# dronefreak/CABiNet

Measured on AMD Instinct MI355X. Metric: 1024x1024 images/sec fwd+bwd (CABiNet-MobileNetV3-Large), higher is better.
Workload: dtype f32; 1 GPU; BASELINE configs[2]: CABiNet-MobileNetV3-Large, 8x3x1024x1024 synthetic 8-class per GPU, fwd + 2x OhemCE + bwd + grad all-reduce + SGD step, HIP CAB/FFM kernels, fp32, random-init (model seed 0, gamma=0.5); per_gpu_batch=8, global_batch=8, n_classes=8, parallelism=dp1, miopen_find_mode=FAST

## Files before the change

cabinet_amd/_lib.py:

```python

from __future__ import annotations

import ctypes
import os
import threading

_PKG_DIR = os.path.dirname(os.path.abspath(__file__))
LIB_PATH = os.path.join(_PKG_DIR, "libcabinet_hip.so")
ABI_VERSION = 8

_c_float_p = ctypes.c_void_p
_INT, _FLT, _SZ, _PTR = ctypes.c_int, ctypes.c_float, ctypes.c_size_t, ctypes.c_void_p

SIGNATURES = {
    "cabinet_abi_version": (_INT, []),
    "cabinet_last_error": (ctypes.c_char_p, []),
    "cabinet_cab_attn_supported": (_INT, [_INT] * 2),
    "cabinet_cab_attn_precision_supported": (_INT, [_INT] * 3),
    "cabinet_cab_attn_fwd_workspace_bytes": (_SZ, [_INT] * 5),
    "cabinet_cab_attn_fwd": (_INT, [_PTR, _PTR, _PTR, _FLT, _INT, _INT, _INT, _INT, _INT, _PTR, _PTR, _PTR, _SZ, _PTR]),
    "cabinet_cab_attn_proj_supported": (_INT, [_INT] * 5),
    "cabinet_cab_attn_proj_fwd": (_INT, [_PTR] * 4 + [_FLT] + [_INT] * 5 + [_PTR] * 3 + [_PTR]),
    "cabinet_cab_attn_bwd_workspace_bytes": (_SZ, [_INT] * 4),
    "cabinet_cab_attn_bwd": (_INT, [_PTR] * 6 + [_FLT] + [_INT] * 4 + [_PTR] * 3 + [_PTR, _SZ, _PTR]),
# ... 20 lines not shown
                            + [_PTR, _SZ, _PTR]),
    "cabinet_cab_qkv_bwd_workspace_bytes": (_SZ, [_INT] * 7 + [_PTR]),
    "cabinet_cab_qkv_bwd": (_INT, [_PTR] * 20 + [_INT] * 7 + [_PTR] + [_INT] + [_PTR] * 9 + [_PTR, _SZ, _PTR]),
    "cabinet_conv1x1_fwd_workspace_bytes": (_SZ, [_INT] * 2),
    "cabinet_conv1x1_fwd": (_INT, [_PTR] * 2 + [_INT] * 4 + [_PTR] + [_PTR, _SZ, _PTR]),
    "cabinet_conv1x1_bias_supported": (_INT, [_INT] * 4),
    "cabinet_conv1x1_bias_fwd": (_INT, [_PTR] * 3 + [_INT] * 4 + [_PTR] + [_PTR, _SZ, _PTR]),
    "cabinet_channel_sum": (_INT, [_PTR] + [_INT] * 3 + [_PTR] + [_PTR]),
    "cabinet_conv1x1_bwd_workspace_bytes": (_SZ, [_INT] * 4),
    "cabinet_conv1x1_bwd": (_INT, [_PTR] * 3 + [_INT] * 4 + [_PTR] * 2 + [_PTR, _SZ, _PTR]),
    "cabinet_bn_act_workspace_bytes": (_SZ, [_INT] * 3),
    "cabinet_bn_act_fwd": (_INT, [_PTR] * 6 + [_INT] * 5 + [_FLT, _FLT] + [_PTR] * 3 + [_PTR, _SZ, _PTR]),
    "cabinet_bn_act_bwd": (_INT, [_PTR] * 6 + [_INT] * 5 + [_PTR] * 3 + [_PTR, _SZ, _PTR]),
    "cabinet_bn_cls_supported": (_INT, [_INT] * 3),
    "cabinet_bn_cls_table_floats": (_INT, [_INT] * 2),
    "cabinet_bn_cls_fwd_workspace_bytes": (_SZ, [_INT] * 3),
    "cabinet_bn_cls_fwd": (_INT, [_PTR] * 8 + [_INT] * 6 + [_FLT, _FLT] + [_PTR] * 2 + [_PTR, _SZ, _PTR]),
    "cabinet_bn_cls_bwd_workspace_bytes": (_SZ, [_INT] * 4),
    "cabinet_bn_cls_bwd": (_INT, [_PTR] * 3 + [_INT] * 6 + [_PTR] * 5 + [_PTR, _SZ, _PTR]),
    "cabinet_gate_act_fwd": (_INT, [_PTR] * 2 + [_INT] * 4 + [_PTR] + [_PTR]),
    "cabinet_gate_act_bwd_workspace_bytes": (_SZ, [_INT] * 3),
    "cabinet_gate_act_bwd": (_INT, [_PTR] * 3 + [_INT] * 4 + [_PTR] * 2 + [_PTR, _SZ, _PTR]),
    "cabinet_bn_dwconv_fwd_workspace_bytes": (_SZ, [_INT] * 4),
    "cabinet_bn_dwconv_fwd": (_INT, [_PTR] * 6 + [_INT] * 8 + [_FLT, _FLT] + [_PTR] * 3 + [_PTR, _SZ, _PTR]),
    "cabinet_bn_dwconv_bwd_workspace_bytes": (_SZ, [_INT] * 6),
    "cabinet_bn_dwconv_bwd": (_INT, [_PTR] * 7 + [_INT] * 8 + [_PTR] * 4 + [_PTR, _SZ, _PTR]),
    "cabinet_stem_conv_fwd": (_INT, [_PTR] * 2 + [_INT] * 3 + [_PTR] + [_PTR]),
    "cabinet_stem_conv_wrw_workspace_bytes": (_SZ, [_INT] * 3),
    "cabinet_stem_conv_wrw": (_INT, [_PTR] * 2 + [_INT] * 3 + [_PTR] + [_PTR, _SZ, _PTR]),
    "cabinet_pwconv_supported": (_INT, [_INT] * 3),
    "cabinet_pwconv_fwd": (_INT, [_PTR] * 2 + [_INT] * 4 + [_PTR] + [_PTR]),
    "cabinet_pwconv_bwd_workspace_bytes": (_SZ, [_INT] * 4),
    "cabinet_pwconv_bwd": (_INT, [_PTR] * 3 + [_INT] * 4 + [_PTR] * 2 + [_PTR, _SZ, _PTR]),
    "cabinet_bn_act_fwd_part": (_INT, [_PTR] * 7 + [_INT] * 6 + [_FLT, _FLT] + [_PTR] * 3 + [_PTR]),
    "cabinet_conv3x3_supported": (_INT, [_INT] * 3),
    "cabinet_conv3x3_tile_blocks": (_INT, [_INT] * 3),
    "cabinet_conv3x3_fwd_workspace_bytes": (_SZ, [_INT] * 6),
    "cabinet_conv3x3_fwd": (_INT, [_PTR] * 3 + [_INT] * 6 + [_PTR] * 2 + [_PTR, _SZ, _PTR]),
    "cabinet_conv3x3_bwd_workspace_bytes": (_SZ, [_INT] * 6),
    "cabinet_conv3x3_bwd": (_INT, [_PTR] * 4 + [_INT] * 6 + [_PTR] * 3 + [_PTR, _SZ, _PTR]),
    "cabinet_dwconv_supported": (_INT, [_INT] * 2),
    "cabinet_dwconv_fwd": (_INT, [_PTR] * 2 + [_INT] * 6 + [_PTR] + [_PTR]),
    "cabinet_dwconv_bwd_workspace_bytes": (_SZ, [_INT] * 6),
    "cabinet_dwconv_bwd": (_INT, [_PTR] * 3 + [_INT] * 6 + [_PTR] * 2 + [_PTR, _SZ, _PTR]),
    "cabinet_cab_local_supported": (_INT, [_INT] * 4),
    "cabinet_cab_local_fwd_workspace_bytes": (_SZ, [_INT] * 4),
    "cabinet_cab_local_bwd_workspace_bytes": (_SZ, [_INT] * 4),
    "cabinet_cab_local_fwd": (_INT, [_PTR] * 3 + [_PTR] * 5 + [_INT] * 5 + [_FLT, _FLT] + [_PTR] * 3 + [_PTR, _SZ, _PTR]),
    "cabinet_cab_local_bwd": (_INT, [_PTR] * 4 + [_PTR] * 3 + [_PTR] * 2 + [_INT] * 5 + [_PTR] * 3 + [_PTR] * 3 + [_PTR, _SZ, _PTR]),
    "cabinet_eval_chip_accum_supported": (_INT, [_INT] * 6),
    "cabinet_eval_chip_accum": (_INT, [_PTR] * 2 + [_INT] * 6 + [_PTR] + [_INT] * 4 + [_PTR] * 2 + [_PTR]),
    "cabinet_eval_scale_merge": (_INT, [_PTR] + [_INT] * 8 + [_PTR] + [_INT] * 2 + [_PTR]),
    "cabinet_eval_argmax_hist": (_INT, [_PTR] * 2 + [_INT] * 5 + [_PTR] * 2 + [_PTR]),
    "cabinet_se_act_bwd_workspace_bytes": (_SZ, [_INT] * 3),
    "cabinet_se_act_bwd_reduce": (_INT, [_PTR] * 8 + [_INT] * 4 + [_PTR] * 2 + [_PTR, _SZ, _PTR]),
    "cabinet_se_act_bwd_coef": (_INT, [_PTR] * 3 + [_INT] * 4 + [_PTR] * 4 + [_PTR]),
    "cabinet_se_act_bwd_dx": (_INT, [_PTR] * 9 + [_INT] * 4 + [_PTR] + [_PTR]),
}

_lock = threading.Lock()
_lib = None


def _preload_hip_runtime():
    import sys

# ... 48 lines not shown
```

cabinet_amd/build.py:

```python

from __future__ import annotations

import argparse
import hashlib
import os
import shutil
import subprocess
import sys
from concurrent.futures import ThreadPoolExecutor

PKG_DIR = os.path.dirname(os.path.abspath(__file__))
CSRC = os.path.join(PKG_DIR, "csrc")
OBJ_DIR = os.path.join(PKG_DIR, "csrc", "build")
LIB_PATH = os.path.join(PKG_DIR, "libcabinet_hip.so")
ARCH = "gfx950"

SOURCES = ["capi.hip", "cab_attn_fwd.hip", "cab_attn_bf16.hip", "cab_attn_bwd.hip", "ffm.hip", "ffm_bwd_fused.hip", "ffm_bwd_adj.hip", "ffm_fwd_fused.hip", "gemm_bf16.hip", "ohem.hip", "cab_local.hip", "cab_local_tiled.hip", "cab_qkv.hip", "cab_qkv_fused.hip", "bn_act.hip", "dwconv.hip", "stem_conv.hip", "pwconv.hip", "small_gemm.hip", "conv3x3_wino.hip", "bn_cls.hip", "eval_tail.hip"]
HEADERS = ["common.hpp", "cab_local.hpp", "cab_qkv.hpp", "blocks.hpp", "act.hpp", "bn_finalize.hpp", os.path.join("..", "..", "include", "cabinet_hip.h")]


def _hipcc():
    for cand in (os.environ.get("HIPCC"), shutil.which("hipcc"), "/opt/rocm/bin/hipcc"):
        if cand and os.path.exists(cand):
            return cand
    raise RuntimeError("hipcc not found: cannot build libcabinet_hip.so")


def _digest(paths):
    h = hashlib.sha256()
    for p in paths:
        with open(p, "rb") as f:
            h.update(f.read())
    return h.hexdigest()


def source_digest():
    paths = [os.path.join(CSRC, s) for s in SOURCES] + [os.path.normpath(os.path.join(CSRC, h)) for h in HEADERS]
    return _digest(paths)


def is_fresh():
    stamp = LIB_PATH + ".stamp"
    if not (os.path.exists(LIB_PATH) and os.path.exists(stamp)):
        return False
    with open(stamp) as f:
        return f.read().strip() == _stamp()


def _stamp():
    return (source_digest() + " " + os.environ.get("CABINET_EXTRA_HIPCC_FLAGS", "").strip()).strip()
# ... 46 lines not shown
```

cabinet_amd/csrc/capi.hip:

```cpp
#include "../../include/cabinet_hip.h"

#include <stdarg.h>
#include <stdint.h>
#include <stdio.h>

#include "blocks.hpp"
#include "cab_local.hpp"
#include "cab_qkv.hpp"
#include "common.hpp"

namespace cabinet {
int attn_fwd_kvsplit(int B, int n);
bool attn_shape_supported(int Kc, int Vc);
hipError_t attn_fwd_dispatch(const float* q, const float* k, const float* v, float scale, int B, int Kc,
                             int Vc, int n, float* ctx, float* lse, float* part_ctx, float* part_lse,
                             int kvsplit, hipStream_t stream);
bool attn_fwd_proj_supported(int B, int Kc, int Vc, int Co, int n);
hipError_t attn_fwd_proj_dispatch(const float* q, const float* k, const float* v, const float* w_out, float scale, int B, int Kc,
                                  int Vc, int Co, int n, float* ctx, float* glob, float* lse, hipStream_t stream);
bool attn_bf16_supported(int Kc, int Vc);
size_t attn_bf16_pack_bytes(int B, int Kc, int Vc, int n, int precision);
hipError_t attn_fwd_bf16_dispatch(const float* q, const float* k, const float* v, float scale, int B, int Kc, int Vc, int n,
                                  float* ctx, float* lse, float* part_ctx, float* part_lse, int kvsplit, void* pack, int precision,
                                  hipStream_t stream);
// ... 53 lines not shown
size_t gate_act_workspace(int rows, int P);
hipError_t gate_act_fwd_run(const float* x, const float* gate, int rows, int P, int act, float* y, hipStream_t stream);
hipError_t gate_act_bwd_run(const float* dy, const float* x, const float* gate, int rows, int P, int act, float* dx,
                            float* dgate, void* ws, hipStream_t stream);
bool bn_cls_supported(int C, int K, int P);
int bn_cls_table_floats(int C, int K);
size_t bn_cls_fwd_workspace(int B, int C, int P);
size_t bn_cls_bwd_workspace(int B, int C, int K, int P);
hipError_t bn_cls_fwd_run(const float* z, const float* conv_part, const float* bn_w, const float* bn_b, float* run_mean, float* run_var,
                          const float* w_cls, const float* bias, int B, int C, int K, int H, int W, int training, float momentum,
                          float eps, float* y, float* tab, void* ws, hipStream_t stream);
hipError_t bn_cls_bwd_run(const float* dy, const float* z, const float* tab, int B, int C, int K, int H, int W, int training, float* dz,
                          float* dbn_w, float* dbn_b, float* dw_cls, float* dbias, void* ws, hipStream_t stream);
bool dwconv_supported(int K, int S);
size_t dwconv_bwd_workspace(int B, int C, int H, int W, int K);
hipError_t dwconv_fwd_run(const float* x, const float* w, int B, int C, int H, int W, int K, int S, float* y,
                          hipStream_t stream);
hipError_t dwconv_bwd_run(const float* dy, const float* x, const float* w, int B, int C, int H, int W, int K, int S,
                          float* dx, float* dw, void* ws, hipStream_t stream);
size_t bn_dwconv_fwd_workspace(int B, int C, int H, int W);
size_t bn_dwconv_bwd_workspace(int B, int C, int H, int W, int K);
hipError_t bn_dwconv_fwd_run(const float* z, const float* bn_w, const float* bn_b, float* run_mean, float* run_var,
                             const float* w, int B, int C, int H, int W, int K, int S, int act, int training,
                             float momentum, float eps, float* y, float* save_mean, float* save_invstd, void* ws,
                             hipStream_t stream);
hipError_t bn_dwconv_bwd_run(const float* dy, const float* z, const float* bn_w, const float* bn_b,
                             const float* save_mean, const float* save_invstd, const float* w, int B, int C, int H,
                             int W, int K, int S, int act, int training, float* dz, float* dbn_w, float* dbn_b,
                             float* dw, void* ws, hipStream_t stream);
size_t stem_conv_wrw_workspace(int B, int H, int W);
hipError_t stem_conv_fwd_run(const float* x, const float* w, int B, int H, int W, float* y, hipStream_t stream);
hipError_t stem_conv_wrw_run(const float* dy, const float* x, int B, int H, int W, float* dw, void* ws,
                             hipStream_t stream);
bool pwconv_supported(int Ci, int Co, int P);
size_t pwconv_bwd_workspace(int B, int Ci, int Co, int P);
hipError_t pwconv_fwd_run(const float* x, const float* w, int B, int Ci, int Co, int P, float* y, hipStream_t stream);
hipError_t pwconv_bwd_run(const float* dy, const float* x, const float* w, int B, int Ci, int Co, int P, float* dx,
                          float* dw, void* ws, hipStream_t stream);
int ohem_blocks(int B, int H, int W);
hipError_t ohem_up_fwd_run(int nh, const float* const* low, const long long* labels, int B, int C, int Hl, int Wl, int H, int W,
                           float thresh, int ignore_lb, float* const* loss_px, float* const* blk_sum, int* const* blk_cnt,
                           hipStream_t stream);
hipError_t ohem_stats_run(const float* blk_sum, const int* blk_cnt, int nheads, int nblk, double* stats, hipStream_t stream);
size_t ohem_up_bwd_workspace(int B, int C, int H, int Wl);
bool ohem_up_supported(int C, int Wl, int W);
hipError_t ohem_up_bwd_run(int nh, const float* const* low, const long long* labels, const float* const* loss_px, int B, int C,
                           int Hl, int Wl, int H, int W, float thresh, int ignore_lb, float coef, float* dlow, void* ws,
                           hipStream_t stream);
struct WinoShape {
    int B, C0, C1, K, H, W;
};
bool conv3x3_supported(int C0, int C1, int K);
bool conv3x3_shape_ok(const WinoShape& s);
int conv3x3_tile_blocks(int B, int H, int W);
size_t conv3x3_fwd_workspace(const WinoShape& s);
size_t conv3x3_bwd_workspace(const WinoShape& s);
hipError_t conv3x3_fwd_run(const WinoShape& s, const float* x0, const float* x1, const float* w, float* y, float* stat_part, void* ws,
                           hipStream_t stream);
hipError_t conv3x3_bwd_run(const WinoShape& s, const float* dy, const float* x0, const float* x1, const float* w, float* dx0,
                           float* dx1, float* dw, void* ws, hipStream_t stream);
int eval_chip_threads(int C, int wl, int cw, int nsrc);
hipError_t eval_chip_accum_run(const float* a, const float* b, int N, int C, int hl, int wl, int ch, int cw, float* dst, int FH,
                               int FW, int y0, int x0, const float* rcp_y, const float* rcp_x, hipStream_t stream);
hipError_t eval_scale_merge_run(const float* prob, int N, int C, int FH, int FW, int hst, int hed, int wst, int wed, float* total,
                                int H, int W, hipStream_t stream);
hipError_t eval_argmax_hist_run(const float* total, const long long* labels, int N, int C, int H, int W, int ignore_lb, long long* hist,
// ... 865 lines not shown
    if (B <= 0 || Ci <= 0 || Co <= 0 || P <= 0) return fail(CABINET_ERR_INVALID_ARG, "%s: non-positive dimension", who);
    if (!cabinet::pwconv_supported(Ci, Co, P))
        return fail(CABINET_ERR_UNSUPPORTED, "%s: Ci=%d, Co=%d (multiples of 8, <= 120, block product <= 8)", who, Ci, Co);
    return CABINET_OK;
}

int cabinet_pwconv_supported(int Ci, int Co, int P) {
    return Ci > 0 && Co > 0 && P > 0 && cabinet::pwconv_supported(Ci, Co, P) ? 1 : 0;
}

int cabinet_pwconv_fwd(const float* x, const float* w, int B, int Ci, int Co, int P, float* y, cabinet_stream_t stream) {
    if (int rc = check_pwconv(B, Ci, Co, P, "pwconv_fwd")) return rc;
    if (!x || !w || !y) return fail(CABINET_ERR_INVALID_ARG, "pwconv_fwd: null tensor pointer");
    return hip_status(cabinet::pwconv_fwd_run(x, w, B, Ci, Co, P, y, static_cast<hipStream_t>(stream)),
                      "pwconv_fwd launch");
}

size_t cabinet_pwconv_bwd_workspace_bytes(int B, int Ci, int Co, int P) {
    if (B <= 0 || Ci <= 0 || Co <= 0 || P <= 0 || !cabinet::pwconv_supported(Ci, Co, P)) return 0;
    return cabinet::pwconv_bwd_workspace(B, Ci, Co, P);
}

int cabinet_pwconv_bwd(const float* dy, const float* x, const float* w, int B, int Ci, int Co, int P, float* dx,
                       float* dw, void* workspace, size_t workspace_bytes, cabinet_stream_t stream) {
    if (int rc = check_pwconv(B, Ci, Co, P, "pwconv_bwd")) return rc;
    if (!dy || !x || !w) return fail(CABINET_ERR_INVALID_ARG, "pwconv_bwd: null tensor pointer");
    const size_t need = cabinet::pwconv_bwd_workspace(B, Ci, Co, P);
    if (dw && (!workspace || workspace_bytes < need))
        return fail(CABINET_ERR_WORKSPACE, "pwconv_bwd: workspace %zu < %zu bytes", workspace_bytes, need);
    return hip_status(cabinet::pwconv_bwd_run(dy, x, w, B, Ci, Co, P, dx, dw, workspace, static_cast<hipStream_t>(stream)),
                      "pwconv_bwd launch");
}

static int check_conv3x3(const cabinet::WinoShape& s, const char* who) {
    if (s.B <= 0 || s.C0 <= 0 || s.C1 < 0 || s.K <= 0 || s.H <= 0 || s.W <= 0)
        return fail(CABINET_ERR_INVALID_ARG, "%s: non-positive dimension", who);
    if (!cabinet::conv3x3_shape_ok(s))
        return fail(CABINET_ERR_UNSUPPORTED,
                    "%s: C0=%d C1=%d Co=%d H=%d W=%d (C0, C1 multiples of 16; Co, C0+C1 multiples of 64; C0 %% 64 == 0 when C1 > 0; "
                    "one image's tensors < 1 GiB)", who, s.C0, s.C1, s.K, s.H, s.W);
    return CABINET_OK;
}

int cabinet_conv3x3_supported(int C0, int C1, int Co) { return cabinet::conv3x3_supported(C0, C1, Co) ? 1 : 0; }

int cabinet_conv3x3_tile_blocks(int B, int H, int W) {
    return B > 0 && H > 0 && W > 0 ? cabinet::conv3x3_tile_blocks(B, H, W) : 0;
}

size_t cabinet_conv3x3_fwd_workspace_bytes(int B, int C0, int C1, int Co, int H, int W) {
    const cabinet::WinoShape s{B, C0, C1, Co, H, W};
    return B > 0 && H > 0 && W > 0 && cabinet::conv3x3_shape_ok(s) ? cabinet::conv3x3_fwd_workspace(s) : 0;
}

int cabinet_conv3x3_fwd(const float* x0, const float* x1, const float* w, int B, int C0, int C1, int Co, int H, int W, float* y,
                        float* bn_part, void* workspace, size_t workspace_bytes, cabinet_stream_t stream) {
    const cabinet::WinoShape s{B, C0, C1, Co, H, W};
    if (int rc = check_conv3x3(s, "conv3x3_fwd")) return rc;
    if (!x0 || !w || !y || (C1 > 0 && !x1)) return fail(CABINET_ERR_INVALID_ARG, "conv3x3_fwd: null tensor pointer");
    CABINET_REQUIRE_ALIGNED("conv3x3_fwd", x0, x1, w, y, bn_part);
    const size_t need = cabinet::conv3x3_fwd_workspace(s);
    if (!workspace || workspace_bytes < need)
        return fail(CABINET_ERR_WORKSPACE, "conv3x3_fwd: workspace %zu < %zu bytes", workspace_bytes, need);
    return hip_status(cabinet::conv3x3_fwd_run(s, x0, C1 > 0 ? x1 : nullptr, w, y, bn_part, workspace, static_cast<hipStream_t>(stream)),
                      "conv3x3_fwd launch");
}
// ... 68 lines not shown
```

cabinet_amd/functional.py:

```python

from __future__ import annotations

import ctypes as _ct

import torch
import torch.nn.functional as F

from . import _lib


def _ptr(t):
    return t.data_ptr() if t is not None else None


def _stream_handle(device):
    return torch.cuda.current_stream(device).cuda_stream


def _workspace(nbytes, device):
    if nbytes == 0:
        return None, 0
    ws = torch.empty(nbytes, dtype=torch.uint8, device=device)
    return ws, nbytes

# ... 1283 lines not shown
        with torch.cuda.device(x.device):
            rc = lib.cabinet_pwconv_fwd(_ptr(x), _ptr(w2), B, Ci, Co, P, _ptr(y), _stream_handle(x.device))
        _lib.check(rc, "cabinet_pwconv_fwd")
        fn_ctx.save_for_backward(x, w2)
        fn_ctx.w_shape = weight.shape
        return y

    @staticmethod
    @torch.amp.custom_bwd(device_type="cuda")
    def backward(fn_ctx, g):
        lib = _lib.load()
        x, w2 = fn_ctx.saved_tensors
        g = _f32c(g)
        Co, Ci = w2.shape
        B, P = x.shape[0], x.shape[2] * x.shape[3]
        dx = torch.empty_like(x) if fn_ctx.needs_input_grad[0] else None
        dw = torch.empty_like(w2) if fn_ctx.needs_input_grad[1] else None
        ws, nbytes = _workspace(lib.cabinet_pwconv_bwd_workspace_bytes(B, Ci, Co, P), x.device)
        with torch.cuda.device(x.device):
            rc = lib.cabinet_pwconv_bwd(_ptr(g), _ptr(x), _ptr(w2), B, Ci, Co, P, _ptr(dx), _ptr(dw), _ptr(ws), nbytes,
                                        _stream_handle(x.device))
        _lib.check(rc, "cabinet_pwconv_bwd")
        return dx, (dw.view(fn_ctx.w_shape) if dw is not None else None)


def pwconv(x, conv):
    if not x.is_cuda:
        raise RuntimeError("pwconv: device tensors only")
    return _PwConv.apply(x, conv.weight)




def eval_chip_accum_supported(logits, chip_size, flip=False):
    if not (logits.is_cuda and logits.dim() == 4 and _lib.available()):
        return False
    _, C, hl, wl = logits.shape
    return bool(_lib.load().cabinet_eval_chip_accum_supported(C, hl, wl, int(chip_size[0]), int(chip_size[1]), int(bool(flip))))


def eval_chip_accum(dst, logits, logits_flipped, chip_size, origin, rcp_y=None, rcp_x=None):
    lib = _lib.load()
    if not (dst.is_cuda and dst.dtype == torch.float32 and dst.is_contiguous()):
        raise RuntimeError("eval_chip_accum: dst must be a dense fp32 device tensor")
    a = _f32c(logits)
    b = _f32c(logits_flipped) if logits_flipped is not None else None
    if b is not None and b.shape != a.shape:
        raise RuntimeError("eval_chip_accum: the flipped chip's logits must have the shape of the chip's")
    N, C, hl, wl = a.shape
    if dst.shape[:2] != (N, C):
        raise RuntimeError(f"eval_chip_accum: dst {tuple(dst.shape)} does not match logits {tuple(a.shape)}")
    FH, FW = dst.shape[2:]
    ry = _f32c(rcp_y) if rcp_y is not None else None
    rx = _f32c(rcp_x) if rcp_x is not None else None
    if (ry is not None and ry.numel() != FH) or (rx is not None and rx.numel() != FW):
        raise RuntimeError("eval_chip_accum: rcp_y / rcp_x must have one entry per row / column of dst")
    dev = dst.device
    with torch.cuda.device(dev):
        rc = lib.cabinet_eval_chip_accum(_ptr(a), _ptr(b), N, C, hl, wl, int(chip_size[0]), int(chip_size[1]), _ptr(dst), FH, FW,
                                         int(origin[0]), int(origin[1]), _ptr(ry), _ptr(rx), _stream_handle(dev))
    _lib.check(rc, "cabinet_eval_chip_accum")
    return dst


def eval_scale_merge_supported(total):
    return bool(total.is_cuda and total.dim() == 4 and _lib.available() and total.shape[0] * total.shape[1] <= 65535
# ... 43 lines not shown
```

cabinet_amd/models/cabinet.py:

```python

from __future__ import annotations

import logging
from pathlib import Path
from typing import Optional, Tuple

import torch
import torch.nn as nn
import torch.nn.functional as F

from .. import functional as _functional
from ..functional import (batched_bn_counters, bn_act, bn_relu_cls, conv1x1, conv1x1_bias_supported, conv3x3, conv3x3_bn_part,
                          conv3x3_supported, ffm_fused, ffm_fused_upsampled, stem_conv, stem_conv_supported)
from .cab import ContextAggregationBlock
from .constants import MODEL_CONFIG, MOBILENETV3_CFGS
from .mobilenetv3 import MobileNetV3

logger = logging.getLogger(__name__)


def _resize(x, size):
    return F.interpolate(x, size=size, mode="bilinear", align_corners=False)


def _is_plain_3x3(conv: nn.Conv2d) -> bool:
    return (conv.kernel_size == (3, 3) and conv.stride == (1, 1) and conv.padding == (1, 1) and conv.dilation == (1, 1) and
            conv.groups == 1 and conv.bias is None and conv.padding_mode == "zeros")


def _conv3x3_bn_relu(conv: nn.Conv2d, bn: nn.BatchNorm2d, x: torch.Tensor, x1: Optional[torch.Tensor] = None) -> torch.Tensor:
    c1 = 0 if x1 is None else x1.shape[1]
    if _functional.CONV3X3_ENABLED and _is_plain_3x3(conv) and conv3x3_supported(x.shape[1], c1, conv.out_channels, x.shape[2], x.shape[3]):
        part = conv3x3_bn_part(x, conv.out_channels) if bn.training else None
        return bn_act(conv3x3(x, conv.weight, x1, part), bn, "relu", conv_part=part)
    return bn_act(conv(x if x1 is None else torch.cat([x, x1], dim=1)), bn, "relu")


def _conv3x3_bn_relu_cls(conv: nn.Conv2d, bn: nn.BatchNorm2d, cls: nn.Conv2d, x: torch.Tensor,
                         x1: Optional[torch.Tensor] = None) -> torch.Tensor:
    c1 = 0 if x1 is None else x1.shape[1]
    if _functional.CONV3X3_ENABLED and _is_plain_3x3(conv) and conv3x3_supported(x.shape[1], c1, conv.out_channels, x.shape[2], x.shape[3]):
        part = conv3x3_bn_part(x, conv.out_channels) if bn.training else None
        return bn_relu_cls(conv3x3(x, conv.weight, x1, part), bn, cls, conv_part=part)
    return bn_relu_cls(conv(x if x1 is None else torch.cat([x, x1], dim=1)), bn, cls)


class ConvBNReLU(nn.Module):

    def __init__(self, in_chan: int, out_chan: int, kernel_size: int = 3, stride: int = 1, padding: int = 1,
                 dilation: int = 1):
        super().__init__()
        self.conv = nn.Conv2d(in_chan, out_chan, kernel_size, stride, padding, dilation=dilation, bias=False)
        self.bn = nn.BatchNorm2d(out_chan)
        self.relu = nn.ReLU(inplace=True)
        self.init_weight()

    def forward(self, x: torch.Tensor) -> torch.Tensor:
        if not x.is_cuda:
            return self.relu(self.bn(self.conv(x)))
        if x.shape[1] == 3 and stem_conv_supported(self.conv):
            return bn_act(stem_conv(x, self.conv), self.bn, "relu")
        return _conv3x3_bn_relu(self.conv, self.bn, x)

    def init_weight(self) -> None:
        nn.init.kaiming_normal_(self.conv.weight, a=1)
        if self.conv.bias is not None:
            nn.init.constant_(self.conv.bias, 0)

# ... 146 lines not shown
```

cabinet_amd/models/mobilenetv3.py:

```python

from __future__ import annotations

import math
from pathlib import Path

import torch
import torch.nn as nn

__all__ = ["MobileNetV3", "InvertedResidual", "SELayer", "HardSwish", "HardSigmoid",
           "mobilenetv3_large", "mobilenetv3_small"]


def _make_divisible(v, divisor, min_value=None):
    floor = divisor if min_value is None else min_value
    rounded = max(floor, int(v + divisor / 2) // divisor * divisor)
    return rounded + divisor if rounded < 0.9 * v else rounded


class HardSigmoid(nn.Module):

    def __init__(self, inplace: bool = True) -> None:
        super().__init__()
        self.relu = nn.ReLU6(inplace=inplace)

# ... 10 lines not shown
    def forward(self, x):
        return x * self.sigmoid(x)


class SELayer(nn.Module):

    def __init__(self, channel, reduction=4):
        super().__init__()
        squeezed = _make_divisible(channel // reduction, 8)
        self.avg_pool = nn.AdaptiveAvgPool2d(1)
        self.fc = nn.Sequential(nn.Linear(channel, squeezed), nn.ReLU(inplace=True),
                                nn.Linear(squeezed, channel), HardSigmoid())

    def gate(self, x):
        n, c = x.shape[:2]
        return self.fc(self.avg_pool(x).view(n, c))

    def forward(self, x):
        n, c = x.shape[:2]
        return x * self.gate(x).view(n, c, 1, 1)


def _act(use_hs):
    return HardSwish() if use_hs else nn.ReLU(inplace=True)


class _FusedSequential(nn.Sequential):

    def forward(self, x, residual=None):
        if not x.is_cuda:
            y = super().forward(x)
            return y if residual is None else residual + y
        from ..functional import (bn_act, bn_act_dwconv, dwconv, dwconv_supported, gate_act, pwconv,
                                  pwconv_supported, se_tail)

        layers = [m for m in self if not isinstance(m, nn.Identity)]

        def act_of(m):
            return "relu" if isinstance(m, nn.ReLU) else "hardswish" if isinstance(m, HardSwish) else None

        i = 0
        while i < len(layers):
            m = layers[i]
            nxt = layers[i + 1] if i + 1 < len(layers) else None
            if isinstance(m, nn.BatchNorm2d) and isinstance(nxt, SELayer):
                act = act_of(layers[i + 2]) if i + 2 < len(layers) else None
                x, i = se_tail(x, m, nxt, act), i + (3 if act else 2)
            elif isinstance(m, nn.BatchNorm2d):
                act = act_of(nxt)
                nxt2 = layers[i + 2] if act and i + 2 < len(layers) else None
                if isinstance(nxt2, nn.Conv2d) and nxt2.groups > 1 and dwconv_supported(nxt2):
                    x, i = bn_act_dwconv(x, m, act, nxt2), i + 3
                else:
                    last = i + (2 if act else 1) >= len(layers)
                    x, i = bn_act(x, m, act, residual if last else None), i + (2 if act else 1)
                    if last:
                        residual = None
            elif isinstance(m, SELayer):
                act = act_of(nxt)
                x, i = gate_act(x, m.gate(x), act), i + (2 if act else 1)
            elif isinstance(m, nn.Conv2d) and m.groups == 1 and pwconv_supported(m, x):
                x, i = pwconv(x, m), i + 1
            elif isinstance(m, nn.Conv2d) and m.groups > 1 and dwconv_supported(m):
                x, i = dwconv(x, m), i + 1
            else:
                x, i = m(x), i + 1
        return x if residual is None else residual + x


def conv_3x3_bn(inp, oup, stride):
    return _FusedSequential(nn.Conv2d(inp, oup, 3, stride, 1, bias=False), nn.BatchNorm2d(oup), HardSwish())


def conv_1x1_bn(inp, oup):
    return _FusedSequential(nn.Conv2d(inp, oup, 1, 1, 0, bias=False), nn.BatchNorm2d(oup), HardSwish())


class InvertedResidual(nn.Module):

    def __init__(self, inp, hidden_dim, oup, kernel_size, stride, use_se, use_hs):
        super().__init__()
        if stride not in (1, 2):
            raise ValueError(f"stride must be 1 or 2, got {stride}")
        self.identity = stride == 1 and inp == oup
        pad = (kernel_size - 1) // 2

        def depthwise():
            return nn.Conv2d(hidden_dim, hidden_dim, kernel_size, stride, pad, groups=hidden_dim, bias=False)

        layers = []
        if inp == hidden_dim:
            layers += [depthwise(), nn.BatchNorm2d(hidden_dim), _act(use_hs)]
            layers += [SELayer(hidden_dim) if use_se else nn.Identity()]
        else:
            layers += [nn.Conv2d(inp, hidden_dim, 1, 1, 0, bias=False), nn.BatchNorm2d(hidden_dim), _act(use_hs)]
            layers += [depthwise(), nn.BatchNorm2d(hidden_dim)]
            layers += [SELayer(hidden_dim) if use_se else nn.Identity(), _act(use_hs)]
# ... 75 lines not shown
```

include/cabinet_hip.h:

```cpp
#ifndef CABINET_HIP_H_
#define CABINET_HIP_H_

#include <stddef.h>

#ifdef __cplusplus
extern "C" {
#endif

#define CABINET_ABI_VERSION 8

#define CABINET_OK 0
#define CABINET_ERR_INVALID_ARG (-1)
#define CABINET_ERR_UNSUPPORTED (-2)
#define CABINET_ERR_WORKSPACE (-3)
#define CABINET_ERR_HIP (-4)

typedef void* cabinet_stream_t;

int cabinet_abi_version(void);
const char* cabinet_last_error(void);

#define CABINET_PREC_FP32 0
#define CABINET_PREC_BF16X3 1
#define CABINET_PREC_BF16X6 2
// ... 181 lines not shown
int cabinet_se_act_bwd_reduce(const float* dy, const float* z, const float* mean, const float* invstd, const float* bn_weight,
                              const float* bn_bias, const float* gate, const float* a2, int B, int C, int P, int act,
                              float* sums, float* da2, void* workspace, size_t workspace_bytes, cabinet_stream_t stream);
int cabinet_se_act_bwd_coef(const float* sums, const float* gate, const float* ds, int B, int C, int P, int training,
                            float* dbn_weight, float* dbn_bias, float* coef, float* ds_over_p, cabinet_stream_t stream);
int cabinet_se_act_bwd_dx(const float* dy, const float* z, const float* mean, const float* invstd, const float* bn_weight,
                          const float* bn_bias, const float* gate, const float* ds_over_p, const float* coef,
                          int B, int C, int P, int act, float* dz, cabinet_stream_t stream);

size_t cabinet_bn_dwconv_fwd_workspace_bytes(int B, int C, int H, int W);
int cabinet_bn_dwconv_fwd(const float* z, const float* bn_weight, const float* bn_bias,
                          float* running_mean, float* running_var, const float* conv_weight,
                          int B, int C, int H, int W, int K, int stride, int act, int training,
                          float momentum, float eps, float* y, float* save_mean, float* save_invstd,
                          void* workspace, size_t workspace_bytes, cabinet_stream_t stream);
size_t cabinet_bn_dwconv_bwd_workspace_bytes(int B, int C, int H, int W, int K, int stride);
int cabinet_bn_dwconv_bwd(const float* dy, const float* z, const float* bn_weight, const float* bn_bias,
                          const float* save_mean, const float* save_invstd, const float* conv_weight,
                          int B, int C, int H, int W, int K, int stride, int act, int training,
                          float* dz, float* dbn_weight, float* dbn_bias, float* dconv_weight,
                          void* workspace, size_t workspace_bytes, cabinet_stream_t stream);

int cabinet_stem_conv_fwd(const float* x, const float* weight, int B, int H, int W, float* y, cabinet_stream_t stream);
size_t cabinet_stem_conv_wrw_workspace_bytes(int B, int H, int W);
int cabinet_stem_conv_wrw(const float* dy, const float* x, int B, int H, int W, float* dw,
                          void* workspace, size_t workspace_bytes, cabinet_stream_t stream);

int cabinet_pwconv_supported(int Ci, int Co, int P);
int cabinet_pwconv_fwd(const float* x, const float* w, int B, int Ci, int Co, int P, float* y, cabinet_stream_t stream);
size_t cabinet_pwconv_bwd_workspace_bytes(int B, int Ci, int Co, int P);
int cabinet_pwconv_bwd(const float* dy, const float* x, const float* w, int B, int Ci, int Co, int P,
                       float* dx, float* dw, void* workspace, size_t workspace_bytes, cabinet_stream_t stream);

int cabinet_conv3x3_supported(int C0, int C1, int Co);
int cabinet_conv3x3_tile_blocks(int B, int H, int W);
size_t cabinet_conv3x3_fwd_workspace_bytes(int B, int C0, int C1, int Co, int H, int W);
int cabinet_conv3x3_fwd(const float* x0, const float* x1, const float* w, int B, int C0, int C1, int Co, int H, int W,
                        float* y, float* bn_part, void* workspace, size_t workspace_bytes, cabinet_stream_t stream);
size_t cabinet_conv3x3_bwd_workspace_bytes(int B, int C0, int C1, int Co, int H, int W);
int cabinet_conv3x3_bwd(const float* dy, const float* x0, const float* x1, const float* w, int B, int C0, int C1, int Co,
                        int H, int W, float* dx0, float* dx1, float* dw,
                        void* workspace, size_t workspace_bytes, cabinet_stream_t stream);

int cabinet_eval_chip_accum_supported(int C, int hl, int wl, int ch, int cw, int flip);
int cabinet_eval_chip_accum(const float* a, const float* b, int N, int C, int hl, int wl, int ch, int cw, float* dst, int FH, int FW,
                            int y0, int x0, const float* rcp_y, const float* rcp_x, cabinet_stream_t stream);
int cabinet_eval_scale_merge(const float* prob, int N, int C, int FH, int FW, int hst, int hed, int wst, int wed, float* total, int H,
                             int W, cabinet_stream_t stream);
int cabinet_eval_argmax_hist(const float* total, const long long* labels, int N, int C, int H, int W, int ignore_lb, long long* hist,
                             unsigned char* pred, cabinet_stream_t stream);

#ifdef __cplusplus
}
#endif
#endif
```

Before: 340.3 images/s.

## Add split-K MFMA weight-gradient kernel for wide pointwise convolutions

Adds a custom HIP kernel for the weight gradient of 1x1 convolutions that pwconv does not cover. It splits the pixel dimension across many workgroups, each accumulating an fp32 MFMA tile into a per-split slab, and a second kernel sums the slabs. Forward and input-gradient still go through MIOpen; only dW replaces MIOpen's wrw path, which is likely slow for tall-skinny reductions at 1024x1024. This adds a workspace of nsplit*Co*Ci floats and an extra reduction launch.

After: 351.2 images/s, median of 6. 3.2% higher.

```diff
diff --git a/cabinet_amd/_lib.py b/cabinet_amd/_lib.py
--- a/cabinet_amd/_lib.py
+++ b/cabinet_amd/_lib.py
@@ -76,6 +76,9 @@
     "cabinet_pwconv_fwd": (_INT, [_PTR] * 2 + [_INT] * 4 + [_PTR] + [_PTR]),
     "cabinet_pwconv_bwd_workspace_bytes": (_SZ, [_INT] * 4),
     "cabinet_pwconv_bwd": (_INT, [_PTR] * 3 + [_INT] * 4 + [_PTR] * 2 + [_PTR, _SZ, _PTR]),
+    "cabinet_pwconv_wide_supported": (_INT, [_INT] * 3),
+    "cabinet_pwconv_wide_wgrad_workspace_bytes": (_SZ, [_INT] * 4),
+    "cabinet_pwconv_wide_wgrad": (_INT, [_PTR] * 2 + [_INT] * 4 + [_PTR] + [_PTR, _SZ, _PTR]),
     "cabinet_bn_act_fwd_part": (_INT, [_PTR] * 7 + [_INT] * 6 + [_FLT, _FLT] + [_PTR] * 3 + [_PTR]),
     "cabinet_conv3x3_supported": (_INT, [_INT] * 3),
     "cabinet_conv3x3_tile_blocks": (_INT, [_INT] * 3),
diff --git a/cabinet_amd/build.py b/cabinet_amd/build.py
--- a/cabinet_amd/build.py
+++ b/cabinet_amd/build.py
@@ -15,7 +15,7 @@
 LIB_PATH = os.path.join(PKG_DIR, "libcabinet_hip.so")
 ARCH = "gfx950"
 
-SOURCES = ["capi.hip", "cab_attn_fwd.hip", "cab_attn_bf16.hip", "cab_attn_bwd.hip", "ffm.hip", "ffm_bwd_fused.hip", "ffm_bwd_adj.hip", "ffm_fwd_fused.hip", "gemm_bf16.hip", "ohem.hip", "cab_local.hip", "cab_local_tiled.hip", "cab_qkv.hip", "cab_qkv_fused.hip", "bn_act.hip", "dwconv.hip", "stem_conv.hip", "pwconv.hip", "small_gemm.hip", "conv3x3_wino.hip", "bn_cls.hip", "eval_tail.hip"]
+SOURCES = ["capi.hip", "cab_attn_fwd.hip", "cab_attn_bf16.hip", "cab_attn_bwd.hip", "ffm.hip", "ffm_bwd_fused.hip", "ffm_bwd_adj.hip", "ffm_fwd_fused.hip", "gemm_bf16.hip", "ohem.hip", "cab_local.hip", "cab_local_tiled.hip", "cab_qkv.hip", "cab_qkv_fused.hip", "bn_act.hip", "dwconv.hip", "stem_conv.hip", "pwconv.hip", "pwconv_wide.hip", "small_gemm.hip", "conv3x3_wino.hip", "bn_cls.hip", "eval_tail.hip"]
 HEADERS = ["common.hpp", "cab_local.hpp", "cab_qkv.hpp", "blocks.hpp", "act.hpp", "bn_finalize.hpp", os.path.join("..", "..", "include", "cabinet_hip.h")]
 
 
diff --git a/cabinet_amd/csrc/capi.hip b/cabinet_amd/csrc/capi.hip
--- a/cabinet_amd/csrc/capi.hip
+++ b/cabinet_amd/csrc/capi.hip
@@ -109,6 +109,10 @@
 hipError_t stem_conv_fwd_run(const float* x, const float* w, int B, int H, int W, float* y, hipStream_t stream);
 hipError_t stem_conv_wrw_run(const float* dy, const float* x, int B, int H, int W, float* dw, void* ws,
                              hipStream_t stream);
+bool pwconv_wide_supported(int Ci, int Co, int P);
+size_t pwconv_wide_wgrad_workspace(int B, int Ci, int Co, int P);
+hipError_t pwconv_wide_wgrad_run(const float* dy, const float* x, int B, int Ci, int Co, int P, float* dw, void* ws,
+                                 hipStream_t stream);
 bool pwconv_supported(int Ci, int Co, int P);
 size_t pwconv_bwd_workspace(int B, int Ci, int Co, int P);
 hipError_t pwconv_fwd_run(const float* x, const float* w, int B, int Ci, int Co, int P, float* y, hipStream_t stream);
@@ -1040,6 +1044,33 @@
                       "pwconv_bwd launch");
 }
 
+int cabinet_pwconv_wide_supported(int Ci, int Co, int P) {
+    return Ci > 0 && Co > 0 && P > 0 && cabinet::pwconv_wide_supported(Ci, Co, P) ? 1 : 0;
+}
+
+size_t cabinet_pwconv_wide_wgrad_workspace_bytes(int B, int Ci, int Co, int P) {
+    if (B <= 0 || Ci <= 0 || Co <= 0 || P <= 0 || !cabinet::pwconv_wide_supported(Ci, Co, P)) return 0;
+    if ((long long)B * ((P + 63) / 64) > (1ll << 30)) return 0;
+    return cabinet::pwconv_wide_wgrad_workspace(B, Ci, Co, P);
+}
+
+int cabinet_pwconv_wide_wgrad(const float* dy, const float* x, int B, int Ci, int Co, int P, float* dw, void* workspace,
+                              size_t workspace_bytes, cabinet_stream_t stream) {
+    if (B <= 0 || Ci <= 0 || Co <= 0 || P <= 0)
+        return fail(CABINET_ERR_INVALID_ARG, "pwconv_wide_wgrad: non-positive dimension");
+    if ((long long)B * ((P + 63) / 64) > (1ll << 30))
+        return fail(CABINET_ERR_UNSUPPORTED, "pwconv_wide_wgrad: B=%d, P=%d: more than 2^30 pixel chunks", B, P);
+    if (!cabinet::pwconv_wide_supported(Ci, Co, P))
+        return fail(CABINET_ERR_UNSUPPORTED, "pwconv_wide_wgrad: Ci=%d, Co=%d, P=%d (multiples of 8, <= 4096, P <= 2^21, max(Ci, Co) * P <= 2^28)",
+                    Ci, Co, P);
+    if (!dy || !x || !dw) return fail(CABINET_ERR_INVALID_ARG, "pwconv_wide_wgrad: null tensor pointer");
+    const size_t need = cabinet::pwconv_wide_wgrad_workspace(B, Ci, Co, P);
+    if (!workspace || workspace_bytes < need)
+        return fail(CABINET_ERR_WORKSPACE, "pwconv_wide_wgrad: workspace %zu < %zu bytes", workspace_bytes, need);
+    return hip_status(cabinet::pwconv_wide_wgrad_run(dy, x, B, Ci, Co, P, dw, workspace, static_cast<hipStream_t>(stream)),
+                      "pwconv_wide_wgrad launch");
+}
+
 static int check_conv3x3(const cabinet::WinoShape& s, const char* who) {
     if (s.B <= 0 || s.C0 <= 0 || s.C1 < 0 || s.K <= 0 || s.H <= 0 || s.W <= 0)
         return fail(CABINET_ERR_INVALID_ARG, "%s: non-positive dimension", who);
diff --git a/cabinet_amd/csrc/pwconv_wide.hip b/cabinet_amd/csrc/pwconv_wide.hip
--- /dev/null
+++ b/cabinet_amd/csrc/pwconv_wide.hip
@@ -0,0 +1,199 @@
+#include "common.hpp"
+
+namespace cabinet {
+
+constexpr int PWW_KC = 64;
+constexpr int PWW_LD = 68;
+constexpr int PWW_TARGET_WG = 512;
+constexpr int PWW_MAX_C = 4096;
+constexpr int PWW_MAX_P = 1 << 21;
+constexpr int PWW_OOB = 0x40000000;
+
+template <int BM, int BN>
+__device__ __forceinline__ void pww_multiply(const float* __restrict__ tl, int kb, int li,
+                                             f32x16 (&acc)[BM][BN]) {
+#pragma unroll
+    for (int s = 0; s < 2; ++s) {
+        f32x4 a[BM], b[BN];
+#pragma unroll
+        for (int i = 0; i < BM; ++i) a[i] = *reinterpret_cast<const f32x4*>(tl + (32 * i + li) * PWW_LD + kb + 8 * s);
+#pragma unroll
+        for (int j = 0; j < BN; ++j)
+            b[j] = *reinterpret_cast<const f32x4*>(tl + (32 * (BM + j) + li) * PWW_LD + kb + 8 * s);
+#pragma unroll
+        for (int q = 0; q < 4; ++q)
+#pragma unroll
+            for (int i = 0; i < BM; ++i)
+#pragma unroll
+                for (int j = 0; j < BN; ++j)
+                    acc[i][j] = mfma32(a[i][q], b[j][q], acc[i][j]);
+    }
+}
+
+template <int BM, int BN>
+__global__ __launch_bounds__(256, 2) void pww_wgrad_kernel(const float* __restrict__ dy, const float* __restrict__ x, int Co,
+                                                        int Ci, int P, int nchunks, int chunks_per_img, int tiles_n,
+                                                        int ntiles, int nsplit, float* __restrict__ slabs) {
+    extern __shared__ __attribute__((aligned(16))) float tl[];
+    constexpr int RPT = 8 * (BM + BN);
+    const int tid = threadIdx.x, lane = tid & 63, wave = tid >> 6, li = lane & 31, h = lane >> 5;
+    const int lin = xcd_chunked_tile(blockIdx.x, gridDim.x);
+    const int split = lin / ntiles, tile = lin - split * ntiles;
+    const int tm = tile / tiles_n, tn = tile - tm * tiles_n;
+    const int co0 = 32 * BM * tm, ci0 = 32 * BN * tn;
+    const int c_begin = (int)((long long)split * nchunks / nsplit), c_end = (int)((long long)(split + 1) * nchunks / nsplit);
+
+    f32x16 acc[BM][BN];
+#pragma unroll
+    for (int i = 0; i < BM; ++i)
+#pragma unroll
+        for (int j = 0; j < BN; ++j)
+#pragma unroll
+            for (int r = 0; r < 16; ++r) acc[i][j][r] = 0.f;
+
+    const int wrow = __builtin_amdgcn_readfirstlane(wave);
+    float v[RPT];
+    auto load = [&](int c) {
+        const int b = c / chunks_per_img, p0 = (c - b * chunks_per_img) * PWW_KC;
+        const int voff = p0 + lane < P ? lane * 4 : PWW_OOB;
+        const int rows_y = Co - co0 - wrow, rows_x = Ci - ci0 - wrow;
+        const buf_rsrc ry = make_rsrc(dy + ((size_t)b * Co + co0 + wrow) * P + p0,
+                                      rows_y > 0 ? (unsigned)(((size_t)(rows_y - 1) * P + (P - p0)) * sizeof(float)) : 0u);
+        const buf_rsrc rx = make_rsrc(x + ((size_t)b * Ci + ci0 + wrow) * P + p0,
+                                      rows_x > 0 ? (unsigned)(((size_t)(rows_x - 1) * P + (P - p0)) * sizeof(float)) : 0u);
+        const int row_bytes = 4 * P * (int)sizeof(float);
+#pragma unroll
+        for (int j = 0; j < 8 * BM; ++j) v[j] = bload(ry, voff, j * row_bytes);
+#pragma unroll
+        for (int j = 0; j < 8 * BN; ++j) v[8 * BM + j] = bload(rx, voff, j * row_bytes);
+    };
+
+    const int kb = 16 * wave + 4 * h;
+    if (c_begin < c_end) load(c_begin);
+    for (int c = c_begin; c < c_end; ++c) {
+        __syncthreads();
+#pragma unroll
+        for (int j = 0; j < RPT; ++j) tl[(wave + 4 * j) * PWW_LD + lane] = v[j];
+        __syncthreads();
+        if (c + 1 < c_end) load(c + 1);
+        pww_multiply<BM, BN>(tl, kb, li, acc);
+    }
+
+    float* slab = slabs + (size_t)split * Co * Ci;
+    const int rr = tid >> 4, c4 = 4 * (tid & 15);
+    const int row_in = (rr & 3) + 8 * (rr >> 2) + 4 * (c4 >> 5), col_in = c4 & 31;
+#pragma unroll
+    for (int i = 0; i < BM; ++i)
+#pragma unroll
+        for (int j = 0; j < BN; ++j) {
+            __syncthreads();
+#pragma unroll
+            for (int r = 0; r < 16; ++r) tl[(wave * 16 + r) * 64 + lane] = acc[i][j][r];
+            __syncthreads();
+            f32x4 t = *reinterpret_cast<const f32x4*>(tl + rr * 64 + c4);
+#pragma unroll
+            for (int w = 1; w < 4; ++w) t += *reinterpret_cast<const f32x4*>(tl + (w * 16 + rr) * 64 + c4);
+            const int co = co0 + 32 * i + row_in, ci = ci0 + 32 * j + col_in;
+            if (co < Co && ci < Ci) *reinterpret_cast<f32x4*>(slab + (size_t)co * Ci + ci) = t;
+        }
+}
+
+template <int Q>
+__global__ __launch_bounds__(32 * Q) void pww_slab_sum_kernel(const float* __restrict__ slabs, int nslab, int count,
+                                                              float* __restrict__ dw) {
+    __shared__ float red[Q][32];
+    const int e = threadIdx.x & 31, q = threadIdx.x >> 5, i = blockIdx.x * 32 + e;
+    float s0 = 0.f, s1 = 0.f, s2 = 0.f, s3 = 0.f;
+    if (i < count) {
+        const float* p = slabs + i;
+        int k = q;
+        for (; k + 3 * Q < nslab; k += 4 * Q) {
+            s0 += p[(size_t)k * count];
+            s1 += p[(size_t)(k + Q) * count];
+            s2 += p[(size_t)(k + 2 * Q) * count];
+            s3 += p[(size_t)(k + 3 * Q) * count];
+        }
+        for (; k < nslab; k += Q) s0 += p[(size_t)k * count];
+    }
+    red[q][e] = (s0 + s1) + (s2 + s3);
+    __syncthreads();
+    if (q == 0 && i < count) {
+        float t = red[0][e];
+#pragma unroll
+        for (int k = 1; k < Q; ++k) t += red[k][e];
+        dw[i] = t;
+    }
+}
+
+struct PwwPlan {
+    int bm, bn, tiles_m, tiles_n, nsplit, nchunks, cpi;
+};
+
+static PwwPlan pww_plan(int B, int Ci, int Co, int P) {
+    static const int shapes[][2] = {{1, 1}, {1, 2}, {2, 1}, {2, 2}, {1, 3}, {3, 1}, {2, 3}, {3, 2}, {1, 4}, {4, 1},
+                                    {2, 4}, {4, 2}, {3, 3}};
+    const int cob = ceil_div(Co, 32), cib = ceil_div(Ci, 32);
+    PwwPlan best{};
+    long best_cost = -1, best_tiles = 0;
+    for (const auto& s : shapes) {
+        const int tm = ceil_div(cob, s[0]), tn = ceil_div(cib, s[1]);
+        const int mfma = 2 * s[0] * s[1], rows = 3 * (s[0] + s[1]);
+        const long tiles = (long)tm * tn, cost = tiles * (mfma > rows ? mfma : rows);
+        if (best_cost < 0 || cost < best_cost || (cost == best_cost && tiles < best_tiles)) {
+            best_cost = cost, best_tiles = tiles;
+            best.bm = s[0], best.bn = s[1], best.tiles_m = tm, best.tiles_n = tn;
+        }
+    }
+    best.cpi = ceil_div(P, PWW_KC);
+    best.nchunks = B * best.cpi;
+    const int ntiles = best.tiles_m * best.tiles_n;
+    int ns = PWW_TARGET_WG / ntiles, cap = best.nchunks / 2;
+    if (ns > cap) ns = cap;
+    best.nsplit = ns < 1 ? 1 : ns;
+    return best;
+}
+
+bool pwconv_wide_supported(int Ci, int Co, int P) {
+    return Ci % 8 == 0 && Co % 8 == 0 && Ci <= PWW_MAX_C && Co <= PWW_MAX_C && P > 0 && P <= PWW_MAX_P &&
+           (size_t)(Ci > Co ? Ci : Co) * P <= ((size_t)1 << 28);
+}
+
+size_t pwconv_wide_wgrad_workspace(int B, int Ci, int Co, int P) {
+    return align_up((size_t)pww_plan(B, Ci, Co, P).nsplit * Co * Ci * sizeof(float), 256);
+}
+
+hipError_t pwconv_wide_wgrad_run(const float* dy, const float* x, int B, int Ci, int Co, int P, float* dw, void* ws,
+                                 hipStream_t stream) {
+    const PwwPlan pl = pww_plan(B, Ci, Co, P);
+    const int ntiles = pl.tiles_m * pl.tiles_n, grid = ntiles * pl.nsplit;
+    const size_t lds = (size_t)32 * (pl.bm + pl.bn) * PWW_LD * sizeof(float);
+    float* slabs = static_cast<float*>(ws);
+#define PWW(BMV, BNV)                                                                                                   \
+    hipLaunchKernelGGL((pww_wgrad_kernel<BMV, BNV>), dim3(grid), dim3(256), lds, stream, dy, x, Co, Ci, P, pl.nchunks,   \
+                       pl.cpi, pl.tiles_n, ntiles, pl.nsplit, slabs)
+    switch (pl.bm * 8 + pl.bn) {
+        case 1 * 8 + 1: PWW(1, 1); break;
+        case 1 * 8 + 2: PWW(1, 2); break;
+        case 2 * 8 + 1: PWW(2, 1); break;
+        case 2 * 8 + 2: PWW(2, 2); break;
+        case 1 * 8 + 3: PWW(1, 3); break;
+        case 3 * 8 + 1: PWW(3, 1); break;
+        case 2 * 8 + 3: PWW(2, 3); break;
+        case 3 * 8 + 2: PWW(3, 2); break;
+        case 1 * 8 + 4: PWW(1, 4); break;
+        case 4 * 8 + 1: PWW(4, 1); break;
+        case 2 * 8 + 4: PWW(2, 4); break;
+        case 4 * 8 + 2: PWW(4, 2); break;
+        default: PWW(3, 3); break;
+    }
+#undef PWW
+    hipError_t e = hipGetLastError();
+    if (e != hipSuccess) return e;
+    if (pl.nsplit >= 128)
+        hipLaunchKernelGGL(pww_slab_sum_kernel<32>, dim3(ceil_div(Co * Ci, 32)), dim3(1024), 0, stream, slabs, pl.nsplit, Co * Ci, dw);
+    else
+        hipLaunchKernelGGL(pww_slab_sum_kernel<8>, dim3(ceil_div(Co * Ci, 32)), dim3(256), 0, stream, slabs, pl.nsplit, Co * Ci, dw);
+    return hipGetLastError();
+}
+
+}
diff --git a/cabinet_amd/functional.py b/cabinet_amd/functional.py
--- a/cabinet_amd/functional.py
+++ b/cabinet_amd/functional.py
@@ -1339,6 +1339,60 @@
 
 
 
+PWCONV_WIDE_ENABLED = _os.environ.get("CABINET_PWCONV_WIDE", "1") != "0"
+
+
+def pwconv_wide_supported(conv, x):
+    if not (PWCONV_WIDE_ENABLED and isinstance(conv, torch.nn.Conv2d) and x.is_cuda and x.dim() == 4):
+        return False
+    if not (conv.kernel_size == (1, 1) and conv.stride == (1, 1) and conv.padding == (0, 0) and conv.groups == 1
+            and conv.bias is None and conv.dilation == (1, 1)):
+        return False
+    if not (torch.is_grad_enabled() and conv.weight.requires_grad) or torch.is_autocast_enabled():
+        return False
+    if x.dtype != torch.float32 or conv.weight.dtype != torch.float32 or x.shape[0] < 1 or x.shape[2] * x.shape[3] < 1:
+        return False
+    return bool(_lib.load().cabinet_pwconv_wide_supported(conv.in_channels, conv.out_channels, x.shape[2] * x.shape[3]))
+
+
+class _PwConvWide(torch.autograd.Function):
+
+    @staticmethod
+    def forward(fn_ctx, x, weight):
+        y = F.conv2d(x, weight)
+        fn_ctx.save_for_backward(x, weight)
+        return y
+
+    @staticmethod
+    def backward(fn_ctx, g):
+        x, w = fn_ctx.saved_tensors
+        dx = None
+        if fn_ctx.needs_input_grad[0]:
+            dx = torch.ops.aten.convolution_backward(g, x, w, None, [1, 1], [0, 0], [1, 1], False, [0, 0], 1,
+                                                     [True, False, False])[0]
+        dw = None
+        if fn_ctx.needs_input_grad[1]:
+            lib = _lib.load()
+            xc, gc = _f32c(x), _f32c(g)
+            Co, Ci = w.shape[0], w.shape[1]
+            B, P = xc.shape[0], xc.shape[2] * xc.shape[3]
+            dw = torch.empty((Co, Ci, 1, 1), dtype=torch.float32, device=x.device)
+            ws, nbytes = _workspace(lib.cabinet_pwconv_wide_wgrad_workspace_bytes(B, Ci, Co, P), x.device)
+            with torch.cuda.device(x.device):
+                rc = lib.cabinet_pwconv_wide_wgrad(_ptr(gc), _ptr(xc), B, Ci, Co, P, _ptr(dw), _ptr(ws), nbytes,
+                                                   _stream_handle(x.device))
+            _lib.check(rc, "cabinet_pwconv_wide_wgrad")
+        return dx, dw
+
+
+def pwconv_wide(x, conv):
+    if not x.is_cuda:
+        raise RuntimeError("pwconv_wide: device tensors only")
+    return _PwConvWide.apply(x, conv.weight)
+
+
+
+
 def eval_chip_accum_supported(logits, chip_size, flip=False):
     if not (logits.is_cuda and logits.dim() == 4 and _lib.available()):
         return False
diff --git a/cabinet_amd/models/cabinet.py b/cabinet_amd/models/cabinet.py
--- a/cabinet_amd/models/cabinet.py
+++ b/cabinet_amd/models/cabinet.py
@@ -11,7 +11,8 @@
 
 from .. import functional as _functional
 from ..functional import (batched_bn_counters, bn_act, bn_relu_cls, conv1x1, conv1x1_bias_supported, conv3x3, conv3x3_bn_part,
-                          conv3x3_supported, ffm_fused, ffm_fused_upsampled, stem_conv, stem_conv_supported)
+                          conv3x3_supported, ffm_fused, ffm_fused_upsampled, pwconv_wide, pwconv_wide_supported, stem_conv,
+                          stem_conv_supported)
 from .cab import ContextAggregationBlock
 from .constants import MODEL_CONFIG, MOBILENETV3_CFGS
 from .mobilenetv3 import MobileNetV3
@@ -33,7 +34,10 @@
     if _functional.CONV3X3_ENABLED and _is_plain_3x3(conv) and conv3x3_supported(x.shape[1], c1, conv.out_channels, x.shape[2], x.shape[3]):
         part = conv3x3_bn_part(x, conv.out_channels) if bn.training else None
         return bn_act(conv3x3(x, conv.weight, x1, part), bn, "relu", conv_part=part)
-    return bn_act(conv(x if x1 is None else torch.cat([x, x1], dim=1)), bn, "relu")
+    xin = x if x1 is None else torch.cat([x, x1], dim=1)
+    if pwconv_wide_supported(conv, xin):
+        return bn_act(pwconv_wide(xin, conv), bn, "relu")
+    return bn_act(conv(xin), bn, "relu")
 
 
 def _conv3x3_bn_relu_cls(conv: nn.Conv2d, bn: nn.BatchNorm2d, cls: nn.Conv2d, x: torch.Tensor,
diff --git a/cabinet_amd/models/mobilenetv3.py b/cabinet_amd/models/mobilenetv3.py
--- a/cabinet_amd/models/mobilenetv3.py
+++ b/cabinet_amd/models/mobilenetv3.py
@@ -66,7 +66,7 @@
             y = super().forward(x)
             return y if residual is None else residual + y
         from ..functional import (bn_act, bn_act_dwconv, dwconv, dwconv_supported, gate_act, pwconv,
-                                  pwconv_supported, se_tail)
+                                  pwconv_supported, pwconv_wide, pwconv_wide_supported, se_tail)
 
         layers = [m for m in self if not isinstance(m, nn.Identity)]
 
@@ -97,6 +97,8 @@
                 x, i = pwconv(x, m), i + 1
             elif isinstance(m, nn.Conv2d) and m.groups > 1 and dwconv_supported(m):
                 x, i = dwconv(x, m), i + 1
+            elif pwconv_wide_supported(m, x):
+                x, i = pwconv_wide(x, m), i + 1
             else:
                 x, i = m(x), i + 1
         return x if residual is None else residual + x
diff --git a/include/cabinet_hip.h b/include/cabinet_hip.h
--- a/include/cabinet_hip.h
+++ b/include/cabinet_hip.h
@@ -237,6 +237,11 @@
 int cabinet_pwconv_bwd(const float* dy, const float* x, const float* w, int B, int Ci, int Co, int P,
                        float* dx, float* dw, void* workspace, size_t workspace_bytes, cabinet_stream_t stream);
 
+int cabinet_pwconv_wide_supported(int Ci, int Co, int P);
+size_t cabinet_pwconv_wide_wgrad_workspace_bytes(int B, int Ci, int Co, int P);
+int cabinet_pwconv_wide_wgrad(const float* dy, const float* x, int B, int Ci, int Co, int P, float* dw,
+                              void* workspace, size_t workspace_bytes, cabinet_stream_t stream);
+
 int cabinet_conv3x3_supported(int C0, int C1, int Co);
 int cabinet_conv3x3_tile_blocks(int B, int H, int W);
 size_t cabinet_conv3x3_fwd_workspace_bytes(int B, int C0, int C1, int Co, int H, int W);
```
